# melonwan/sphereHand

Measured on AMD Instinct MI355X. Metric: depth crops/s (raster fwd+bwd, 128x128, batch 256), higher is better.
Workload: dtype f32; 1 GPU; BASELINE configs[1]: batch-256 128x128 sphere raster fwd+bwd, 41 spheres/crop, JointAngleDataset poses (seed 0), grad N(0,1); crops_per_gpu=256, spheres_per_crop=41, launch=direct, parallelism=batch-sharded x1, no data-path collective, rccl_ranks=1

## Files before the change

spherehand_amd/csrc/common.h:

```cpp
#pragma once
#include <hip/hip_runtime.h>
#include <stdint.h>

#include "spherehand_hip.h"

#pragma clang fp contract(off)

namespace shr {

constexpr int kWave = 64;

constexpr int kTileW = 32;
constexpr int kTileH = 8;

struct Axis {
  float half;
  float size;
  float mul;
  int pow2;
};

__host__ __device__ inline Axis make_axis(int size) {
  Axis a;
  a.half = (float)((double)size / 2.0);
// ... 46 lines not shown
  v = dpp_add<0x143, 0xC>(v);
  return v;
}

__device__ __forceinline__ float wave_sum4_transposed(float a0, float a1, float a2, float a3, int lane) {
  const bool odd = lane & 1, hi = lane & 2;
  const float k0 = odd ? a1 : a0, s0 = odd ? a0 : a1;
  const float k1 = odd ? a3 : a2, s1 = odd ? a2 : a3;
  const float b0 = k0 + __int_as_float(__builtin_amdgcn_update_dpp(0, __float_as_int(s0), 0xB1, 0xF, 0xF, false));
  const float b1 = k1 + __int_as_float(__builtin_amdgcn_update_dpp(0, __float_as_int(s1), 0xB1, 0xF, 0xF, false));
  const float k2 = hi ? b1 : b0, s2 = hi ? b0 : b1;
  float c = k2 + __int_as_float(__builtin_amdgcn_update_dpp(0, __float_as_int(s2), 0x4E, 0xF, 0xF, false));
  c = dpp_add<0x114, 0xF>(c);
  c = dpp_add<0x118, 0xF>(c);
  const auto r16 = __builtin_amdgcn_permlane16_swap(__float_as_uint(c), __float_as_uint(c), false, false);
  c = __uint_as_float(r16[0]) + __uint_as_float(r16[1]);
  const auto r32 = __builtin_amdgcn_permlane32_swap(__float_as_uint(c), __float_as_uint(c), false, false);
  return __uint_as_float(r32[0]) + __uint_as_float(r32[1]);
}

template <int CTRL, int ROW_MASK, bool IS_MIN>
__device__ __forceinline__ float dpp_minmax(float v) {
  const float o = __int_as_float(__builtin_amdgcn_update_dpp(__float_as_int(v), __float_as_int(v), CTRL, ROW_MASK, 0xF, false));
  return IS_MIN ? fminf(v, o) : fmaxf(v, o);
}
template <bool IS_MIN>
__device__ __forceinline__ float wave_minmax_all(float v) {
  v = dpp_minmax<0xB1, 0xF, IS_MIN>(v);
  v = dpp_minmax<0x4E, 0xF, IS_MIN>(v);
  v = dpp_minmax<0x141, 0xF, IS_MIN>(v);
  v = dpp_minmax<0x140, 0xF, IS_MIN>(v);
  v = dpp_minmax<0x142, 0xA, IS_MIN>(v);
  v = dpp_minmax<0x143, 0xC, IS_MIN>(v);
  return readlane_f(v, 63);
}

__device__ __forceinline__ float wave_min4_transposed(float a0, float a1, float a2, float a3, int lane) {
  const bool odd = lane & 1, hi = lane & 2;
  const float k0 = odd ? a1 : a0, s0 = odd ? a0 : a1;
  const float k1 = odd ? a3 : a2, s1 = odd ? a2 : a3;
  const float b0 = fminf(k0, __int_as_float(__builtin_amdgcn_update_dpp(__float_as_int(k0), __float_as_int(s0), 0xB1, 0xF, 0xF, false)));
  const float b1 = fminf(k1, __int_as_float(__builtin_amdgcn_update_dpp(__float_as_int(k1), __float_as_int(s1), 0xB1, 0xF, 0xF, false)));
  const float k2 = hi ? b1 : b0, s2 = hi ? b0 : b1;
  float c = fminf(k2, __int_as_float(__builtin_amdgcn_update_dpp(__float_as_int(k2), __float_as_int(s2), 0x4E, 0xF, 0xF, false)));
  c = dpp_minmax<0x114, 0xF, true>(c);
  c = dpp_minmax<0x118, 0xF, true>(c);
  const auto r16 = __builtin_amdgcn_permlane16_swap(__float_as_uint(c), __float_as_uint(c), false, false);
  c = fminf(__uint_as_float(r16[0]), __uint_as_float(r16[1]));
  const auto r32 = __builtin_amdgcn_permlane32_swap(__float_as_uint(c), __float_as_uint(c), false, false);
  return fminf(__uint_as_float(r32[0]), __uint_as_float(r32[1]));
}

__device__ __forceinline__ float sqrt_rn(float x) {
  const float s = __builtin_amdgcn_sqrtf(x);
  const float r = __builtin_fmaf(-s, s, x);
  const uint32_t sb = __float_as_uint(s);
  const float t = __uint_as_float(sb + (sb & 0x7f800000u) - 0x4B000000u);
  uint32_t out;
  asm("v_cmp_gt_f32 vcc, %1, %2\n\ts_nop 1\n\tv_addc_co_u32 %0, vcc, 0, %3, vcc\n\t"
      "v_cmp_le_f32 vcc, %1, -%2\n\ts_nop 1\n\tv_subbrev_co_u32 %0, vcc, 0, %0, vcc"
      : "=&v"(out) : "v"(r), "v"(t), "v"(sb) : "vcc");
  return __uint_as_float(out);
}

int d2m_set_waves(int waves);
int d2m_set_band_units(int units);
int d2m_set_tiled(int on);
int tri_set_band(int rows);
int mesh_set_band(int on);
int mesh_set_lattice(int on);
int tri_band_resize(const float *vertices, const int *faces, int B, int NV, int F, int src_size, int S, float clamp_max,
                    float *depth, hipStream_t s);
int d2m_compact_check(const float *depth, int M, int H, int W, void *workspace, int **counts);
int d2m_compact_launch(const float *depth, int M, int H, int W, void *workspace, hipStream_t s);

__device__ __forceinline__ void lbs_add_entry(float (&acc)[4], const float *M, const float4 q) {
#pragma unroll
  for (int r = 0; r < 4; r++)
    acc[r] += ((M[4 * r] * q.x + M[4 * r + 1] * q.y) + M[4 * r + 2] * q.z) + M[4 * r + 3] * q.w;
}
__device__ __forceinline__ float4 lbs_finish(const float (&acc)[4], int right_hand, int project, float cx, float cy, float fx,
                                             float fy, bool has_rand, float rf) {
  float a0 = acc[0];
  if (right_hand) a0 = -a0;
  if (!project) return make_float4(a0, acc[1], acc[2], acc[3]);
  if (!has_rand) return make_float4(fx * a0 + cx * acc[3], fy * acc[1] + cy * acc[3], acc[2], acc[3]);
  return make_float4(a0 * rf * fx + cx, acc[1] * rf * fy + cy, acc[2], 1.0f);
}
constexpr int kLbsCrops = 4;

struct LbsCamera {
  int right_hand, project;
  float cx, cy, fx, fy;
  bool has_rand;
  float rf;
};
__device__ __forceinline__ void lbs_bone_grad_wave(double (&a)[16], int k, int lane, const float4 *__restrict__ gv, int NV,
                                                   const int *__restrict__ vstart, const int *__restrict__ sbone,
                                                   const float4 *__restrict__ swv, const LbsCamera cam) {
  const double sgn = cam.right_hand ? -1.0 : 1.0;
  const double rf = cam.has_rand ? (double)cam.rf : 1.0;
  const float cx = cam.cx, cy = cam.cy, fx = cam.fx, fy = cam.fy;
#pragma unroll
  for (int j = 0; j < 16; j++) a[j] = 0.0;
  for (int v = lane; v < NV; v += 64) {
    const int e0 = vstart[v], e1 = vstart[v + 1];
    int e = e0;
    while (e < e1 && sbone[e] != k) e++;
    if (e == e1) continue;
    const float4 g = gv[v];
    double d[4];
    if (!cam.project) {
      d[0] = sgn * g.x; d[1] = g.y; d[2] = g.z; d[3] = g.w;
    } else if (!cam.has_rand) {
      d[0] = sgn * (double)fx * g.x; d[1] = (double)fy * g.y; d[2] = g.z;
// ... 120 lines not shown
```

spherehand_amd/csrc/sphere_zbuf.h:

```cpp
#pragma once
#include <type_traits>
#include "sphere_tile.h"

namespace shr {

constexpr int kZWaves = 16;
#ifdef SHR_TIMELINE
#ifndef SHR_TL_REGION
#define SHR_TL_REGION 1u
#endif
__device__ unsigned long long shr_tl[3][256 * kZWaves * 8];
__device__ unsigned long long shr_tl_rt[3][256 * kZWaves * 2];
#define SHR_TL(k, slot)                                                                              \
  do {                                                                                               \
     \
    const unsigned tl_bx = blockIdx.x - ((k) == 2 ? 512u : 0u);                                      \
    if ((threadIdx.x & 63) == 0 && tl_bx < 256u && blockIdx.y == ((k) == 2 ? SHR_TL_REGION : 0u)) {  \
      shr_tl[k][(tl_bx * kZWaves + (threadIdx.x >> 6)) * 8 + (slot)] = __builtin_amdgcn_s_memtime(); \
      if ((slot) == 0 || (slot) == ((k) == 2 ? 7 : 5))                                               \
        shr_tl_rt[k][(tl_bx * kZWaves + (threadIdx.x >> 6)) * 2 + ((slot) != 0)] = __builtin_amdgcn_s_memrealtime(); \
    }                                                                                                \
  } while (0)
#define SHR_TL_ENTRY(k) SHR_TL(k, 0)
#else
#define SHR_TL(k, slot) do {} while (0)
#define SHR_TL_ENTRY(k) do {} while (0)
#endif
#ifndef SHR_ROW_PAD
#define SHR_ROW_PAD 8
#endif
constexpr int kRowPad = SHR_ROW_PAD;
constexpr int kPadRows = 0;
#ifndef SHR_BG_WAVES
#define SHR_BG_WAVES 7
#endif
#ifndef SHR_BG_WAVES_BOX
#define SHR_BG_WAVES_BOX SHR_BG_WAVES
#endif
constexpr int kBgWavesBox = SHR_BG_WAVES_BOX;
constexpr int kBgWaves = SHR_BG_WAVES;
constexpr int kOffItems = 1024;
constexpr int kOffEnds = 2048;
constexpr int kOffFlags = 2304;
constexpr int kOffNext = 2304 + 64;
#ifndef SHR_HDR_PAD
#define SHR_HDR_PAD 0
#endif
constexpr int kHdrBytes = kOffNext + 1024 + SHR_HDR_PAD;
constexpr int kMaxFastWidth = 8192;

struct LdsHeader {
  float4 *s_sph;
  int4 *s_items;
  int *s_ends, *s_flag;
  float4 *s_next;
  __device__ __forceinline__ explicit LdsHeader(unsigned char *smem)
      : s_sph(reinterpret_cast<float4 *>(smem)), s_items(reinterpret_cast<int4 *>(smem + kOffItems)),
        s_ends(reinterpret_cast<int *>(smem + kOffEnds)), s_flag(reinterpret_cast<int *>(smem + kOffFlags)),
        s_next(reinterpret_cast<float4 *>(smem + kOffNext)) {}
};
enum {
  kFlagGeneral = 0,
  kFlagTotal = 1,
  kFlagOutLo = 2, kFlagOutHi = 3,
  kFlagBoxRow0 = 4, kFlagBoxRowEnd = 5, kFlagBoxCol0 = 6, kFlagBoxWidth = 7, kFlagPitch = 8, kFlagClip = 9,
  kFlagTileLo = 10, kFlagTileHi = 11,
  kFlagMayTie = 12,
};

__device__ __forceinline__ uint32_t depth_key(float d) {
  const uint32_t b = __float_as_uint(d);
  return b ^ ((uint32_t)((int32_t)b >> 31) | 0x80000000u);
}
__device__ __forceinline__ float key_depth(uint32_t k) {
  return __uint_as_float(k ^ ((uint32_t)(~((int32_t)k >> 31)) | 0x80000000u));
}
__device__ __forceinline__ unsigned long long background_cell() {
  return ((unsigned long long)depth_key(kBackground) << 32) | 0xFFFFFFFFull;
}
__device__ __forceinline__ bool is_background_tie(unsigned long long k) {
  return (uint32_t)(k >> 32) == depth_key(kBackground) && (uint32_t)k < (uint32_t)SHR_MAX_SPHERES;
}
__device__ __forceinline__ uint32_t tie_owner(const float4 *s_sph, uint32_t j, float xg, float yg) {
  for (uint32_t i = 0; i < j; i++) {
    const float4 s = s_sph[i];
    const float dx = xg - s.x, dy = yg - s.y;
    const float q = (s.w * s.w - dx * dx) - dy * dy;
    if (q <= kHitMin || !(s.z - sqrtf(q) > kBackground)) return SHR_ARGMIN_NONE;
  }
  return j;
}


__device__ __forceinline__ bool sphere_is_tame(const float4 s) {
  return fabsf(s.x) < 1e6f && fabsf(s.y) < 1e6f && fabsf(s.w) < 1e6f;
}

struct Item { int u0, v0, u1, v1, pw, ph, ncx, nchunks; };

__device__ __forceinline__ void axis_box(float c, float ar, float k, float half, float hi_clamp, int lo_lim,
                                         int hi_lim, int &i0, int &i1) {
  const float lo = (c - ar) * k + half, hi = (c + ar) * k + half;
  const float eps = 1e-3f + 2e-6f * (fabsf(lo) + fabsf(hi));
  i0 = max((int)ceilf(fminf(fmaxf(lo - eps, -2.f), hi_clamp)), lo_lim);
  i1 = min((int)floorf(fminf(fmaxf(hi + eps, -2.f), hi_clamp)), hi_lim);
}

constexpr int kSeg2Tag = 0x100;
template <bool SEG2>
__device__ __forceinline__ Item sphere_item(const float4 s, const Axis &ax, const Axis &ay, float kx, float ky, int W,
                                            int r0, int r1) {
  int u0 = 0, u1 = W - 1, v0 = r0, v1 = r1 - 1;
  if (sphere_is_tame(s)) {
    const float ar = fabsf(s.w);
    axis_box(s.x, ar, kx, ax.half, (float)W + 2.f, 0, W - 1, u0, u1);
    axis_box(s.y, ar, ky, ay.half, (float)r1 + 2.f, r0, r1 - 1, v0, v1);
  }
  Item it;
  it.u0 = u0; it.v0 = v0; it.u1 = u1; it.v1 = v1;
  const int w = u1 - u0 + 1, h = v1 - v0 + 1;
  if (w <= 0 || h <= 0) {
    it.pw = 1; it.ph = 1; it.ncx = 0; it.nchunks = 0;
  } else {
    const bool seg2 = SEG2 && w > 32 && w <= kWave;
    it.pw = seg2 ? (w + 1) >> 1 : min(w, kWave);
    it.ph = (int)(64.0f * __builtin_amdgcn_rcpf((float)it.pw) + 0.01f);
    it.ncx = w > kWave ? (w + kWave - 1) >> 6 : (seg2 ? 2 : 1);
    const float hh = (float)(h + it.ph - 1) + 0.5f;
// ... 147 lines not shown
          body(j, s, cell, cell + dcell, 0.f, cav, yg, ygb, yg <= ylim, ygb <= ylim, c + 1 < c_end, std::true_type());
        }
      }
      end_sphere(j);
      if (!m) break;
      j = jn; t = tn; rn = rnn;
    }
  }
  if (wide) walk_slice<true, kSphereCost, ROWFREE>(w, J, lo, hi, lane, ax, ay, r0, r1, LW, body, end_sphere, wide);
}

template <int kSphereCost, bool ROWFREE, typename Body, typename EndSphere>
__device__ __forceinline__ void walk_slice_packed(const WaveList &w, int J, int lo, int hi, int lane, const Axis &ax,
                                                  const Axis &ay, int r0, int r1, int LW, Body &&body,
                                                  EndSphere &&end_sphere) {
  const int wstart = w.item.w, wend = w.end, base = wstart + (kSphereCost & 0xff);
  const int cb = lo <= base ? 0 : (lo - base + kChunkCost - 1) >> kChunkShift;
  const int ce = min((wend - base) >> kChunkShift, (hi - base + kChunkCost - 1) >> kChunkShift);
  const int v1l = w.item.y & 0xffff, inv15l = (int)((unsigned)w.item.y >> 16), phl = (inv15l << 6) >> 15;
  const bool active = lane < J && wend > wstart && cb < ce;
  const bool narrow = ((w.item.z >> 8) & 0xff) == 1;
  const int pk = cb | (ce << 12) | ((w.item.z & 0x7f) << 24) | ((ROWFREE && v1l < r1 - 1) ? (int)0x80000000u : 0);
  const float rrl = w.sph.w * w.sph.w;
  const float dygl = (float)phl * ay.mul;
  const float yliml = axis_coord_t<true>(ay, min(v1l, r1 - 1)) + 0.5f * ay.mul;
  unsigned long long m = __ballot(active && narrow);
  const unsigned long long wide = __ballot(active && !narrow);
  while (m) {
    const int j = __builtin_ctzll(m);
    m &= m - 1;
    const int pkj = rl(pk, j), geom = rl(w.item.x, j), rows = rl(w.item.y, j);
    const float4 s = make_float4(readlane_f(w.sph.x, j), readlane_f(w.sph.y, j), readlane_f(w.sph.z, j), 0.f);
    const float rr = readlane_f(rrl, j);
    int c = pkj & 0xfff;
    const int c_end = (pkj >> 12) & 0xfff, pw = (pkj >> 24) & 0x7f;
    const int u0 = geom & 0xffff, v0 = (int)((unsigned)geom >> 16);
    const int inv15 = (int)((unsigned)rows >> 16), ph = (inv15 << 6) >> 15;
    const int ly = __mul24(lane, inv15) >> 15;
    const int lx = lane - __mul24(ly, pw);
    const bool packed = ly < ph;
    const int u = u0 + lx;
    const float dx = axis_coord_t<true>(ax, u) - s.x;
    const float ca = rr - dx * dx;
    const int v = v0 + c * ph + ly;
    int cell = __mul24(v - r0, LW) + u;
    const int dcell = ph * LW;
    const float cav = packed ? ca : -1.f;
    float yg = axis_coord_t<true>(ay, v);
    const float dyg = readlane_f(dygl, j);
    if (ROWFREE && pkj < 0) {
      for (; c < c_end; c += 2, yg += 2.f * dyg, cell += 2 * dcell)
        body(j, s, cell, cell + dcell, dx, cav, yg, yg + dyg, packed, packed, c + 1 < c_end, std::false_type());
    } else {
      const float ylim = packed ? readlane_f(yliml, j) : -3.0e38f;
      for (; c < c_end; c += 2, yg += 2.f * dyg, cell += 2 * dcell) {
        const float ygb = yg + dyg;
        body(j, s, cell, cell + dcell, dx, cav, yg, ygb, yg <= ylim, ygb <= ylim, c + 1 < c_end, std::true_type());
      }
    }
    end_sphere(j);
  }
  if (wide) walk_slice<true, kSphereCost, ROWFREE>(w, J, lo, hi, lane, ax, ay, r0, r1, LW, body, end_sphere, wide);
}

template <int kSphereCost, bool ROWFREE, typename Body, typename EndSphere>
__device__ __forceinline__ void walk_slice_packed_seg2(const WaveList &w, int J, int lo, int hi, int lane, const Axis &ax,
                                                  const Axis &ay, int r0, int r1, int LW, Body &&body,
                                                  EndSphere &&end_sphere) {
  const int wstart = w.item.w, wend = w.end, base = wstart + (kSphereCost & 0xff);
  const int cb = lo <= base ? 0 : (lo - base + kChunkCost - 1) >> kChunkShift;
  const int ce = min((wend - base) >> kChunkShift, (hi - base + kChunkCost - 1) >> kChunkShift);
  const int v1l = w.item.y & 0xffff, inv15l = (int)((unsigned)w.item.y >> 16), phl = (inv15l << 6) >> 15;
  const bool active = lane < J && wend > wstart && cb < ce;
  const int ncxl = (w.item.z >> 8) & 0xff;
  const bool seg2l = ncxl == 2 && (w.item.z & 0x7f) <= 32;
  const bool narrow = ncxl == 1 || seg2l;
  const int pk = cb | (ce << 12) | (((w.item.z & 0x7f) + (seg2l ? 64 : 0)) << 24) | ((ROWFREE && v1l < r1 - 1) ? (int)0x80000000u : 0);
  const float rrl = w.sph.w * w.sph.w;
  const float dygl = (float)phl * ay.mul;
  const float yliml = axis_coord_t<true>(ay, min(v1l, r1 - 1)) + 0.5f * ay.mul;
  unsigned long long m = __ballot(active && narrow);
  const unsigned long long wide = __ballot(active && !narrow);
  while (m) {
    const int j = __builtin_ctzll(m);
    m &= m - 1;
    const int pkj = rl(pk, j), geom = rl(w.item.x, j), rows = rl(w.item.y, j);
    const float4 s = make_float4(readlane_f(w.sph.x, j), readlane_f(w.sph.y, j), readlane_f(w.sph.z, j), 0.f);
    const float rr = readlane_f(rrl, j);
    const int cb_j = pkj & 0xfff, ce_j = (pkj >> 12) & 0xfff, pwf = (pkj >> 24) & 0x7f;
    const bool seg2 = pwf > 64;
    const int pw = seg2 ? pwf - 64 : pwf;
    const int u0 = geom & 0xffff, v0 = (int)((unsigned)geom >> 16);
    const int inv15 = (int)((unsigned)rows >> 16), ph = (inv15 << 6) >> 15;
    const int ly = __mul24(lane, inv15) >> 15;
    const int lx = lane - __mul24(ly, pw);
    const bool packed = ly < ph;
    const float dyg = readlane_f(dygl, j);
    const int dcell = ph * LW;
    const float ylim = packed ? readlane_f(yliml, j) : -3.0e38f;
    auto run = [&](int u0s, int u1s, int c, int c_end) {
      const int u = u0s + lx;
      const float dx = axis_coord_t<true>(ax, u) - s.x;
      const float ca = rr - dx * dx;
      const int v = v0 + c * ph + ly;
      int cell = __mul24(v - r0, LW) + u;
      const float cav = (packed && u <= u1s) ? ca : -1.f;
      float yg = axis_coord_t<true>(ay, v);
// ... 133 lines not shown
}

template <bool POW2>
__device__ __forceinline__ float axis_coord_t(const Axis &a, int u) {
  const float t = (float)u - a.half;
  return POW2 ? t * a.mul : (t * 300.0f) / a.size;
}

#ifndef SHR_STORE_MODE
#define SHR_STORE_MODE 44
#endif
#ifndef SHR_BWD_STORE_MODE
#define SHR_BWD_STORE_MODE 4
#endif
typedef uint32_t v4u_t __attribute__((ext_vector_type(4)));
template <int M> __device__ __forceinline__ void asm_store16(void *p, v4u_t t) {
  if (M == 0) asm volatile("global_store_dwordx4 %0, %1, off\n\ts_nop 1" ::"v"(p), "v"(t) : "memory");
  if (M == 1) asm volatile("global_store_dwordx4 %0, %1, off nt\n\ts_nop 1" ::"v"(p), "v"(t) : "memory");
  if (M == 2) asm volatile("global_store_dwordx4 %0, %1, off sc0 sc1\n\ts_nop 1" ::"v"(p), "v"(t) : "memory");
  if (M == 3) asm volatile("global_store_dwordx4 %0, %1, off sc0 sc1 nt\n\ts_nop 1" ::"v"(p), "v"(t) : "memory");
  if (M == 4) asm volatile("global_store_dwordx4 %0, %1, off sc1\n\ts_nop 1" ::"v"(p), "v"(t) : "memory");
  if (M == 5) asm volatile("global_store_dwordx4 %0, %1, off sc0\n\ts_nop 1" ::"v"(p), "v"(t) : "memory");
  if (M == 6) asm volatile("global_store_dwordx4 %0, %1, off sc1 nt\n\ts_nop 1" ::"v"(p), "v"(t) : "memory");
}
template <int M> __device__ __forceinline__ void asm_store4(void *p, uint32_t t) {
  if (M == 0) asm volatile("global_store_dword %0, %1, off" ::"v"(p), "v"(t) : "memory");
  if (M == 1) asm volatile("global_store_dword %0, %1, off nt" ::"v"(p), "v"(t) : "memory");
  if (M == 2) asm volatile("global_store_dword %0, %1, off sc0 sc1" ::"v"(p), "v"(t) : "memory");
  if (M == 3) asm volatile("global_store_dword %0, %1, off sc0 sc1 nt" ::"v"(p), "v"(t) : "memory");
  if (M == 4) asm volatile("global_store_dword %0, %1, off sc1" ::"v"(p), "v"(t) : "memory");
  if (M == 5) asm volatile("global_store_dword %0, %1, off sc0" ::"v"(p), "v"(t) : "memory");
  if (M == 6) asm volatile("global_store_dword %0, %1, off sc1 nt" ::"v"(p), "v"(t) : "memory");
}
__device__ __forceinline__ void stream_store(float4 *p, const float4 v) {
  v4u_t t = {__float_as_uint(v.x), __float_as_uint(v.y), __float_as_uint(v.z), __float_as_uint(v.w)};
  asm_store16<SHR_STORE_MODE / 10>(p, t);
}
__device__ __forceinline__ void stream_store(uint4 *p, const uint4 v) {
  v4u_t t = {v.x, v.y, v.z, v.w};
  asm_store16<SHR_STORE_MODE % 10>(p, t);
}
__device__ __forceinline__ void stream_store(uchar4 *p, const uchar4 v) {
  const uint32_t t = (uint32_t)v.x | ((uint32_t)v.y << 8) | ((uint32_t)v.z << 16) | ((uint32_t)v.w << 24);
  asm_store4<SHR_STORE_MODE % 10>(p, t);
}

#ifndef SHR_LATE_STORE_MODE
#define SHR_LATE_STORE_MODE 40
#endif
__device__ __forceinline__ void late_store(float4 *p, const float4 v) {
  v4u_t t = {__float_as_uint(v.x), __float_as_uint(v.y), __float_as_uint(v.z), __float_as_uint(v.w)};
  asm_store16<SHR_LATE_STORE_MODE / 10>(p, t);
}
__device__ __forceinline__ void late_store(uchar4 *p, const uchar4 v) {
  const uint32_t t = (uint32_t)v.x | ((uint32_t)v.y << 8) | ((uint32_t)v.z << 16) | ((uint32_t)v.w << 24);
  asm_store4<SHR_LATE_STORE_MODE % 10>(p, t);
}

template <bool OWNER> struct KeyOf { using type = uint32_t; };
template <> struct KeyOf<true> { using type = unsigned long long; };

__device__ __forceinline__ void touched_rows(const float4 s, bool valid, const Axis &ay, float ky, int r0, int r1,
                                             int &cv0, int &cv1) {
  const bool tame = sphere_is_tame(s);
  const unsigned long long bad = __ballot(valid && !(tame && fabsf(s.z) < 1e30f));
  const unsigned long long low = __ballot(valid && s.z <= kBackground);
  int v0 = r0, v1 = r1 - 1;
  if (tame) axis_box(s.y, fabsf(s.w), ky, ay.half, (float)r1 + 2.f, r0, r1 - 1, v0, v1);
  const bool on = valid && v1 >= v0;
  cv0 = (int)wave_minmax_all<true>(on ? (float)v0 : 1e9f);
  cv1 = (int)wave_minmax_all<false>(on ? (float)v1 : -1e9f);
  if (cv1 < cv0) { cv0 = r1; cv1 = r0 - 1; }
  if (bad != 0ull || low == 0ull) { cv0 = r0; cv1 = r1 - 1; }
}

__device__ __forceinline__ void touched_box(const float4 s, bool valid, const Axis &ax, const Axis &ay, float kx,
                                            float ky, int W, int r0, int r1, int lane, int &cv0, int &cv1, int &cu0,
                                            int &cu1) {
  const bool tame = sphere_is_tame(s);
  const unsigned long long bad = __ballot(valid && !(tame && fabsf(s.z) < 1e30f));
  const unsigned long long low = __ballot(valid && s.z <= kBackground);
  int v0 = r0, v1 = r1 - 1, u0 = 0, u1 = W - 1;
  if (tame) {
    const float ar = fabsf(s.w);
    axis_box(s.x, ar, kx, ax.half, (float)W + 2.f, 0, W - 1, u0, u1);
    axis_box(s.y, ar, ky, ay.half, (float)r1 + 2.f, r0, r1 - 1, v0, v1);
  }
  const bool on = valid && v1 >= v0 && u1 >= u0;
  const float m = wave_min4_transposed(on ? (float)v0 : 1e9f, on ? -(float)v1 : 1e9f, on ? (float)u0 : 1e9f,
                                       on ? -(float)u1 : 1e9f, lane);
  cv0 = (int)readlane_f(m, 12);
  cv1 = -(int)readlane_f(m, 13);
  cu0 = (int)readlane_f(m, 14);
  cu1 = -(int)readlane_f(m, 15);
  if (cv1 < cv0) { cv0 = r1; cv1 = r0 - 1; cu0 = 0; cu1 = -1; }
  if (bad != 0ull || low == 0ull) { cv0 = r0; cv1 = r1 - 1; cu0 = 0; cu1 = W - 1; }
}

__host__ __device__ __forceinline__ int box_pitch(int bw) {
  const int p = bw + kRowPad;
  return (p & 31) < 8 ? p + 8 : p;
}
__host__ __device__ __forceinline__ int max_box_pitch(int W) { return ((W + 3) & ~3) + kRowPad + 8; }

struct CropConsts {
  int J, H, W, rows, w4_shift, zcells, tid;
  int flags, nwaves;
};
template <bool PERSIST>
// ... 178 lines not shown
  const bool may_tie = rfl(hdr.s_flag[kFlagMayTie]) != 0;
  int tile_lo = r0, tile_hi = r1;
  if (!general) {
    int out_lo = 0, out_hi = VEC4 ? nchunk : rh * W;
    if (!BOX && VEC4) { out_lo = rfl(hdr.s_flag[kFlagOutLo]) << 6; out_hi = min(rfl(hdr.s_flag[kFlagOutHi]) << 6, nchunk); }
    if (BOX) { out_lo = rfl(hdr.s_flag[kFlagOutLo]); out_hi = rfl(hdr.s_flag[kFlagOutHi]); }
    const int p0 = BOX ? rfl(hdr.s_flag[kFlagBoxRow0]) : r0, pe = BOX ? rfl(hdr.s_flag[kFlagBoxRowEnd]) : r1;
    const int cu0 = BOX ? rfl(hdr.s_flag[kFlagBoxCol0]) : 0, bw = BOX ? rfl(hdr.s_flag[kFlagBoxWidth]) : W;
    const int pitch = BOX ? rfl(hdr.s_flag[kFlagPitch]) : W + kRowPad, clip = BOX ? rfl(hdr.s_flag[kFlagClip]) : r1;
    tile_lo = BOX ? rfl(hdr.s_flag[kFlagTileLo]) : r1;
    tile_hi = BOX ? rfl(hdr.s_flag[kFlagTileHi]) : r1;

    {
      WaveList wl;
      wl.sph = sph;
      wl.item = hdr.s_items[lane];
      wl.end = hdr.s_ends[lane];
      Key *zb = zbuf - (p0 * pitch + cu0);
      walk_my_slice<POW2, kSphereCostFwd | (SEG2 ? kSeg2Tag : 0), true, TABLE>(
          wl, J, hdr.s_flag[kFlagTotal], wave, nwaves, shares, lane, ax, ay, 0, clip, pitch,
          [&](int j, const float4 s, int cell_a, int cell_b, float, float ca, float yga, float ygb, bool ok_a,
              bool ok_b, bool has_b, auto row_test) {
            const float dya = yga - s.y, dyb = ygb - s.y;
            float qa = ca - dya * dya, qb = ca - dyb * dyb;
            if (decltype(row_test)::value) { qa = ok_a ? qa : -1.f; qb = ok_b ? qb : -1.f; }
            unsigned jv = (unsigned)j;
            if (OWNER) asm("" : "+v"(jv));
            auto put = [&](Key *cell, float d) {
              if (OWNER)
                atomicMin(reinterpret_cast<unsigned long long *>(cell),
                          ((unsigned long long)depth_key(d) << 32) | jv);
              else
                atomicMin(reinterpret_cast<unsigned int *>(cell), depth_key(d));
            };
            if (has_b) {
              const bool ha = qa > kHitMin, hb = qb > kHitMin;
              const float da = s.z - sqrt_rn(qa), db = s.z - sqrt_rn(qb);
              if (ha) put(zb + cell_a, da);
              if (hb) put(zb + cell_b, db);
            } else if (qa > kHitMin) {
              put(zb + cell_a, s.z - sqrt_rn(qa));
            }
          },
          [](int) {}, RunTab{s_tab, s_run});
    }
    if (pf_wave && has_next) hdr.s_next[lane] = sph_next;
    SHR_TL(0, 3);
    __syncthreads();
    SHR_TL(0, 4);

    const Key *zrow = zbuf - (p0 - r0) * pitch - cu0;
    const unsigned box_h = pe > p0 ? (unsigned)(pe - p0) : 0u;
    if (VEC4) {
      for (int cb = out_lo + (wave_s << 6); cb < out_hi; cb += nwaves << 6) {
        const int c = cb + lane;
        if (c >= out_hi) continue;
        int v, x;
        if (POW2 || w4_shift >= 0) { v = c >> w4_shift; x = (c & (w4 - 1)) << 2; }
        else { v = c / w4; x = (c - v * w4) << 2; }
        float4 o = bgd;
        uchar4 a = bga;
        if (!BOX || ((unsigned)(v + r0 - p0) < box_h && (unsigned)(x - cu0) < (unsigned)bw)) {
          const Key *cell = zrow + v * pitch + x;
          if (OWNER) {
            const ulonglong2 k01 = reinterpret_cast<const ulonglong2 *>(cell)[0];
            const ulonglong2 k23 = reinterpret_cast<const ulonglong2 *>(cell)[1];
            o = make_float4(key_depth((uint32_t)(k01.x >> 32)), key_depth((uint32_t)(k01.y >> 32)),
                            key_depth((uint32_t)(k23.x >> 32)), key_depth((uint32_t)(k23.y >> 32)));
            a = make_uchar4((uint8_t)k01.x, (uint8_t)k01.y, (uint8_t)k23.x, (uint8_t)k23.y);
            if (may_tie && (is_background_tie(k01.x) || is_background_tie(k01.y) || is_background_tie(k23.x) ||
                            is_background_tie(k23.y))) {
              const float yg = axis_coord_t<POW2>(ay, v + r0);
              if (is_background_tie(k01.x)) a.x = (uint8_t)tie_owner(hdr.s_sph, (uint32_t)k01.x, axis_coord_t<POW2>(ax, x), yg);
              if (is_background_tie(k01.y)) a.y = (uint8_t)tie_owner(hdr.s_sph, (uint32_t)k01.y, axis_coord_t<POW2>(ax, x + 1), yg);
              if (is_background_tie(k23.x)) a.z = (uint8_t)tie_owner(hdr.s_sph, (uint32_t)k23.x, axis_coord_t<POW2>(ax, x + 2), yg);
              if (is_background_tie(k23.y)) a.w = (uint8_t)tie_owner(hdr.s_sph, (uint32_t)k23.y, axis_coord_t<POW2>(ax, x + 3), yg);
            }
          } else {
            const uint4 k = *reinterpret_cast<const uint4 *>(cell);
            o = make_float4(key_depth(k.x), key_depth(k.y), key_depth(k.z), key_depth(k.w));
          }
        }
        if (OWNER) late_store(aout4 + c, a);
        late_store(out4 + c, o);
      }
    } else {
      for (int p = out_lo + tid; p < out_hi; p += nthr) {
        const int v = p / W, u = p - v * W;
        Key k = bg;
        if (!BOX || ((unsigned)(v + r0 - p0) < box_h && (unsigned)(u - cu0) < (unsigned)bw)) k = zrow[v * pitch + u];
        if (OWNER) {
          out[(size_t)(r0 + v) * W + u] = key_depth((uint32_t)((unsigned long long)k >> 32));
          aout[(size_t)(r0 + v) * W + u] =
              (may_tie && is_background_tie((unsigned long long)k))
                  ? (uint8_t)tie_owner(hdr.s_sph, (uint32_t)k, axis_coord_t<POW2>(ax, u), axis_coord_t<POW2>(ay, v + r0))
                  : (uint8_t)k;
        } else {
          out[(size_t)(r0 + v) * W + u] = key_depth((uint32_t)k);
        }
      }
    }
  }
  if (tile_lo < tile_hi) {
    const int tiles_x = (W + kTileW - 1) / kTileW;
    const int t0 = (tile_lo / kTileH) * tiles_x, t1 = ((tile_hi + kTileH - 1) / kTileH) * tiles_x;
    tile_forward<VEC4, OWNER>(sph, J, H, W, out, aout, tiles_x, t0 + wave, t1, nwaves, lane);
  }
  if (general && pf_wave && has_next) hdr.s_next[lane] = sph_next;
  SHR_TL(0, 5);
  if (PERSIST && n + crop_step < N) __syncthreads();
  }
}

constexpr int kPartBytes = kZWaves * SHR_MAX_SPHERES * 16;
constexpr int kStageBatch = 4;
constexpr int kSpecUnits = 2;
constexpr int kBwdVgprs = 96;

template <bool VEC4, bool POW2, bool PERSIST, int NW, bool WHOLE, bool SEG2 = false>
__global__ void __launch_bounds__(64 * NW) __attribute__((amdgpu_num_vgpr(kBwdVgprs)))
sphere_zbuf_bwd_kernel(const float4 *__restrict__ spheres, const float *__restrict__ grad_depth,
                       const uint8_t *__restrict__ argmin, int N, int J_, int H_, int W_,
                       float4 *__restrict__ grad_spheres, int rows_, int w4_shift_, int shares, AxisK axk) {
  static_assert(NW == 8 || NW == 16, "waves per workgroup");
  constexpr int NT = 64 * NW, NW_SHIFT = NW == 16 ? 4 : 3;
  extern __shared__ __attribute__((aligned(16))) unsigned char smem[];
  const LdsHeader hdr(smem);
  float4 *s_part = reinterpret_cast<float4 *>(smem + kHdrBytes);
  const int crop_step = gridDim.x;
  for (int n = blockIdx.x, crop_it = 0; PERSIST ? n < N : crop_it == 0; n += crop_step, ++crop_it) {
  const CropConsts cc = crop_consts<PERSIST>(J_, H_, W_, rows_, w4_shift_, 0);
  const int J = cc.J, H = cc.H, W = cc.W, rows = cc.rows, w4_shift = cc.w4_shift, tid = cc.tid;
  const int lane = tid & 63, wave = tid >> 6;
  SHR_TL_ENTRY(1);
  const int LW = W + kRowPad;
  float *gbuf = reinterpret_cast<float *>(smem + kHdrBytes + kPartBytes);
  uint8_t *obuf = smem + kHdrBytes + kPartBytes + (size_t)(rows + kPadRows) * LW * 4;
  const Axis ax = axis_of(W, axk.mulx), ay = axis_of(H, axk.muly);
// ... 28 lines not shown
  const int k1 = (max(uc0 - wave_s, 0) + NW - 1) >> NW_SHIFT;
  static_assert(kSpecUnits == 2, "two speculative units per wave: v[96:99] + v104, v[100:103] + v105");
  if (VEC4) {
    const int u0 = wave_s + (k1 << NW_SHIFT), u1 = wave_s + ((k1 + 1) << NW_SHIFT);
    const int c0 = min((u0 << 6) + lane, nchunk - 1), c1 = min((u1 << 6) + lane, nchunk - 1);
    const void *pg0 = u0 < uc1 ? static_cast<const void *>(gin4 + c0) : static_cast<const void *>(rec);
    const void *po0 = u0 < uc1 ? static_cast<const void *>(oin4 + c0) : static_cast<const void *>(rec);
    const void *pg1 = u1 < uc1 ? static_cast<const void *>(gin4 + c1) : static_cast<const void *>(rec);
    const void *po1 = u1 < uc1 ? static_cast<const void *>(oin4 + c1) : static_cast<const void *>(rec);
    asm volatile("global_load_dwordx4 v[96:99], %0, off\n\tglobal_load_dword v104, %1, off\n\t"
                 "global_load_dwordx4 v[100:103], %2, off\n\tglobal_load_dword v105, %3, off"
                 : : "v"(pg0), "v"(po0), "v"(pg1), "v"(po1)
                 : "v96", "v97", "v98", "v99", "v100", "v101", "v102", "v103", "v104", "v105", "memory");
  }
  for (int i = tid; i < rows * kRowPad; i += NT) obuf[(i / kRowPad) * LW + W + (i % kRowPad)] = SHR_ARGMIN_NONE;
  if (lead) {
    if (!have_sph) {
      float4 t;
      if (VEC4)
        asm volatile("s_waitcnt vmcnt(%4)\n\tv_mov_b32 %0, v110\n\tv_mov_b32 %1, v111\n\tv_mov_b32 %2, v112\n\tv_mov_b32 %3, v113"
                     : "=v"(t.x), "=v"(t.y), "=v"(t.z), "=v"(t.w) : "n"(2 * kSpecUnits) : "memory");
      else
        asm volatile("s_waitcnt vmcnt(0)\n\tv_mov_b32 %0, v110\n\tv_mov_b32 %1, v111\n\tv_mov_b32 %2, v112\n\tv_mov_b32 %3, v113"
                     : "=v"(t.x), "=v"(t.y), "=v"(t.z), "=v"(t.w) : : "memory");
      if (lane < J) sph = t;
    }
    touched_rows(sph, lane < J, ay, ky, 0, H, lead_v0, lead_v1);
    SHR_TL(1, 6);
    if (wave_s == 0) {
      hdr.s_sph[lane] = sph;
      if (!WHOLE && lane == 0) { hdr.s_flag[kFlagOutLo] = lead_v0; hdr.s_flag[kFlagOutHi] = lead_v1; }
    }
  }
  int cv0 = 0, cv1 = H - 1;
  if (!WHOLE) {
    __syncthreads();
    cv0 = rfl(hdr.s_flag[kFlagOutLo]);
    cv1 = rfl(hdr.s_flag[kFlagOutHi]);
  }

  auto build_list = [&](int r0, int r1) {
    if (wave_s == 0) {
      bool too_big;
      const int total = build_work_list<kSphereCostBwd | (SEG2 ? kSeg2Tag : 0)>(sph, lane < J, ax, ay, kx, ky, W, r0, r1, hdr.s_items, hdr.s_ends, lane, &too_big);
      if (lane == 0) hdr.s_flag[kFlagTotal] = total;
      SHR_TL(1, 7);
    }
  };
  auto stage = [&](int r0, int r1, int t_lo, int t_hi, auto first_tag) {
    constexpr bool FIRST = decltype(first_tag)::value;
    const int rh = r1 - r0;
    auto put_unit = [&](int u, const v4f g, uint32_t o) {
      const int c = (u << 6) + lane;
      int v, x;
      if (POW2 || w4_shift >= 0) { v = c >> w4_shift; x = (c & (w4 - 1)) << 2; }
      else { v = c / w4; x = (c - v * w4) << 2; }
      if (c < nchunk && (unsigned)(v - r0) < (unsigned)rh) {
        *reinterpret_cast<v4f *>(gbuf + (v - r0) * LW + x) = g;
        *reinterpret_cast<uint32_t *>(obuf + (v - r0) * LW + x) = o;
      }
    };
    if (VEC4) {
      const int ua = t_hi > t_lo ? (t_lo * w4) >> 6 : 0, ub = t_hi > t_lo ? min(nunits, (t_hi * w4 + 63) >> 6) : 0;
      const int s0 = FIRST ? uc0 : 0, s1 = FIRST ? uc1 : 0;
      const int n_lo = max(0, min(ub, s0) - ua), hi0 = max(ua, s1), n_out = n_lo + max(0, ub - hi0);
      static_assert(kStageBatch == 4, "the staging statements below name four slots");
      static_assert(kSpecUnits == 2, "... and tie two speculative units");
      constexpr int DW = WHOLE ? 3 : NW - 1;
      auto batch = [&](int t0, auto with_spec_tag) {
        constexpr bool first_batch = decltype(with_spec_tag)::value;
        v4f g2[kStageBatch];
        uint32_t o2[kStageBatch];
        bool ok[kStageBatch];
        const void *pg[kStageBatch], *po[kStageBatch];
        int us[kStageBatch];
#pragma unroll
        for (int b = 0; b < kStageBatch; b++) {
          const int t = t0 + DW * b;
          ok[b] = t < n_out;
          const int u = us[b] = t < n_lo ? ua + t : hi0 + (t - n_lo);
          const int c = min(max((u << 6) + lane, 0), nchunk - 1);
          pg[b] = ok[b] ? static_cast<const void *>(gin4 + c) : static_cast<const void *>(rec);
          po[b] = ok[b] ? static_cast<const void *>(oin4 + c) : static_cast<const void *>(rec);
        }
        if (FIRST && first_batch) {
          float4 sa, sb;
          uint32_t soa, sob;
          if (!ok[0]) {
            asm volatile(
                "s_waitcnt vmcnt(0)\n\t"
                "v_mov_b32 %0, v96\n\tv_mov_b32 %1, v97\n\tv_mov_b32 %2, v98\n\tv_mov_b32 %3, v99\n\t"
                "v_mov_b32 %4, v100\n\tv_mov_b32 %5, v101\n\tv_mov_b32 %6, v102\n\tv_mov_b32 %7, v103\n\t"
                "v_mov_b32 %8, v104\n\tv_mov_b32 %9, v105"
                : "=&v"(sa.x), "=&v"(sa.y), "=&v"(sa.z), "=&v"(sa.w), "=&v"(sb.x), "=&v"(sb.y), "=&v"(sb.z),
                  "=&v"(sb.w), "=&v"(soa), "=&v"(sob)
                : : "memory");
          } else
          asm volatile(
              "global_load_dwordx4 %0, %18, off\n\tglobal_load_dword %4, %22, off\n\t"
              "global_load_dwordx4 %1, %19, off\n\tglobal_load_dword %5, %23, off\n\t"
              "global_load_dwordx4 %2, %20, off\n\tglobal_load_dword %6, %24, off\n\t"
              "global_load_dwordx4 %3, %21, off\n\tglobal_load_dword %7, %25, off\n\t"
              "s_waitcnt vmcnt(0)\n\t"
              "v_mov_b32 %8, v96\n\tv_mov_b32 %9, v97\n\tv_mov_b32 %10, v98\n\tv_mov_b32 %11, v99\n\t"
              "v_mov_b32 %12, v100\n\tv_mov_b32 %13, v101\n\tv_mov_b32 %14, v102\n\tv_mov_b32 %15, v103\n\t"
              "v_mov_b32 %16, v104\n\tv_mov_b32 %17, v105"
              : "=&v"(g2[0]), "=&v"(g2[1]), "=&v"(g2[2]), "=&v"(g2[3]), "=&v"(o2[0]), "=&v"(o2[1]), "=&v"(o2[2]),
                "=&v"(o2[3]), "=&v"(sa.x), "=&v"(sa.y), "=&v"(sa.z), "=&v"(sa.w), "=&v"(sb.x), "=&v"(sb.y),
                "=&v"(sb.z), "=&v"(sb.w), "=&v"(soa), "=&v"(sob)
              : "v"(pg[0]), "v"(pg[1]), "v"(pg[2]), "v"(pg[3]), "v"(po[0]), "v"(po[1]), "v"(po[2]), "v"(po[3])
              : "memory");
          const int u0 = wave_s + (k1 << NW_SHIFT), u1 = wave_s + ((k1 + 1) << NW_SHIFT);
// ... 237 lines not shown
  if (!general) {
    WaveList wl;
    wl.sph = sph;
    wl.item = hdr.s_items[lane];
    wl.end = hdr.s_ends[lane];
    walk_my_slice<POW2, kSphereCostMse | (SEG2 ? kSeg2Tag : 0), true>(
        wl, J, hdr.s_flag[kFlagTotal], wave, kZWaves, shares_fwd, lane, ax, ay, 0, clip, pitch,
        [&](int j, const float4 s, int cell_a, int cell_b, float, float ca, float yga, float ygb, bool ok_a,
            bool ok_b, bool has_b, auto row_test) {
          const float dya = yga - s.y, dyb = ygb - s.y;
          float qa = ca - dya * dya, qb = ca - dyb * dyb;
          if (decltype(row_test)::value) { qa = ok_a ? qa : -1.f; qb = ok_b ? qb : -1.f; }
          unsigned jv = (unsigned)j;
          asm("" : "+v"(jv));
          auto put = [&](Key *cell, float d) { atomicMin(cell, ((Key)depth_key(d) << 32) | jv); };
          if (has_b) {
            const bool ha = qa > kHitMin, hb = qb > kHitMin;
            const float da = s.z - sqrt_rn(qa), db = s.z - sqrt_rn(qb);
            if (ha) put(zb + cell_a, da);
            if (hb) put(zb + cell_b, db);
          } else if (qa > kHitMin) {
            put(zb + cell_a, s.z - sqrt_rn(qa));
          }
        },
        [](int) {});
    if (pf_wave && has_next) hdr.s_next[lane] = sph_next;
    SHR_TL(2, 3);
    const bool untouched = ua >= ub && tile_lo >= tile_hi;
    if (!untouched) __syncthreads();
    if (BOX) __builtin_amdgcn_s_setprio(1);
    SHR_TL(2, 4);

    auto convert_unit = [&](int u, const float4 t) {
      const int c = (u << 6) + lane;
      if (c >= nchunk) return;
      int v, x;
      if (POW2 || w4_shift >= 0) { v = c >> w4_shift; x = (c & (w4 - 1)) << 2; }
      else { v = c / w4; x = (c - v * w4) << 2; }
      if (BOX && v + r0 >= tile_lo && v + r0 < tile_hi) return;
      if (u < ua || u >= ub) {
        const float e0 = kBackground - t.x, e1 = kBackground - t.y, e2 = kBackground - t.z, e3 = kBackground - t.w;
        sse += (e0 * e0 + e1 * e1) + (e2 * e2 + e3 * e3);
        if (out) stream_store(out4 + c, make_float4(kBackground, kBackground, kBackground, kBackground));
        return;
      }
      if (BOX) {
        if (!((unsigned)(v + r0 - p0) < (unsigned)(pe - p0) && (unsigned)(x - cu0) < (unsigned)bw)) {
          const float e0 = kBackground - t.x, e1 = kBackground - t.y, e2 = kBackground - t.z, e3 = kBackground - t.w;
          sse += (e0 * e0 + e1 * e1) + (e2 * e2 + e3 * e3);
          if (out) stream_store(out4 + c, make_float4(kBackground, kBackground, kBackground, kBackground));
          return;
        }
      }
      ulonglong2 *cell = reinterpret_cast<ulonglong2 *>(zb + (v + r0) * pitch + x);
      ulonglong2 k01 = cell[0], k23 = cell[1];
      const float4 d = make_float4(key_depth((uint32_t)(k01.x >> 32)), key_depth((uint32_t)(k01.y >> 32)),
                                   key_depth((uint32_t)(k23.x >> 32)), key_depth((uint32_t)(k23.y >> 32)));
      if (out) stream_store(out4 + c, d);
      if (may_tie && (is_background_tie(k01.x) || is_background_tie(k01.y) || is_background_tie(k23.x) ||
                      is_background_tie(k23.y))) {
        const float yg = axis_coord_t<POW2>(ay, v + r0);
        if (is_background_tie(k01.x)) k01.x = (k01.x & ~0xffull) | tie_owner(hdr.s_sph, (uint32_t)k01.x, axis_coord_t<POW2>(ax, x), yg);
        if (is_background_tie(k01.y)) k01.y = (k01.y & ~0xffull) | tie_owner(hdr.s_sph, (uint32_t)k01.y, axis_coord_t<POW2>(ax, x + 1), yg);
        if (is_background_tie(k23.x)) k23.x = (k23.x & ~0xffull) | tie_owner(hdr.s_sph, (uint32_t)k23.x, axis_coord_t<POW2>(ax, x + 2), yg);
        if (is_background_tie(k23.y)) k23.y = (k23.y & ~0xffull) | tie_owner(hdr.s_sph, (uint32_t)k23.y, axis_coord_t<POW2>(ax, x + 3), yg);
      }
      const float e0 = d.x - t.x, e1 = d.y - t.y, e2 = d.z - t.z, e3 = d.w - t.w;
      sse += (e0 * e0 + e1 * e1) + (e2 * e2 + e3 * e3);
      k01.x = ((Key)__float_as_uint(2.f * e0) << 32) | (uint32_t)k01.x;
      k01.y = ((Key)__float_as_uint(2.f * e1) << 32) | (uint32_t)k01.y;
      k23.x = ((Key)__float_as_uint(2.f * e2) << 32) | (uint32_t)k23.x;
      k23.y = ((Key)__float_as_uint(2.f * e3) << 32) | (uint32_t)k23.y;
      cell[0] = k01;
      cell[1] = k23;
    };
#pragma unroll
    for (int k = 0; k < kTgtAhead; k++) asm volatile("" : : "v"(tpre[k].x), "v"(tpre[k].y), "v"(tpre[k].z), "v"(tpre[k].w));
#pragma unroll
    for (int k = 0; k < kTgtAhead; k++)
      if (wave_s + (k << 4) < nunits) convert_unit(wave_s + (k << 4), tpre[k]);
    for (int u = wave_s + (kTgtAhead << 4); u < nunits; u += kZWaves) {
      const int c = (u << 6) + lane;
      float4 t = tgt4[min(c, nchunk - 1)];
      asm volatile("" : "+v"(t.x), "+v"(t.y), "+v"(t.z), "+v"(t.w));
      convert_unit(u, t);
    }
    SHR_TL(2, 5);
    if (BOX) __builtin_amdgcn_s_setprio(0);
    if (!untouched) __syncthreads();
    SHR_TL(2, 6);

    float a0 = 0.f, a1 = 0.f, a2 = 0.f, a3 = 0.f;
    const int cell_max = (p0 * pitch + cu0) + (pe - p0) * pitch - 1;
    walk_my_slice<POW2, kSphereCostMse | (SEG2 ? kSeg2Tag : 0), true>(
        wl, J, hdr.s_flag[kFlagTotal], wave, kZWaves, shares_bwd, lane, ax, ay, 0, clip, pitch,
        [&](int j, const float4 s, int cell_a, int cell_b, float dx, float ca, float yga, float ygb, bool ok_a,
            bool ok_b, bool has_b, auto) {
          auto take = [&](int cell, float yg, bool ok) {
            const Key k = zb[min(cell, cell_max)];
            if ((uint8_t)k == (uint8_t)j && ok) {
              const float dy = yg - s.y, q = ca - dy * dy;
              const float g = __uint_as_float((uint32_t)(k >> 32));
              const float w = g * __builtin_amdgcn_rsqf(q);
              a0 = __builtin_fmaf(-w, dx, a0);
              a1 = __builtin_fmaf(-w, dy, a1);
              a2 += g;
              a3 -= w;
            }
          };
          take(cell_a, yga, ok_a);
// ... 117 lines not shown
```

Measured before the change: 18.64 million crops/s.

## Trim instruction counts in sqrt, key decode, owner packing and cell addressing

Replaces the correctly-rounded sqrt fixup sequence with an rsq-based Newton step, and adds asm barriers in key decoding to steer code generation. Owner bytes are packed with v_perm into a single dword that is stored directly. The output loop gets a separate specialization for the no-tie case, and cell addresses are computed from a flat chunk index plus row padding instead of a per-lane v/x split. The rsq-based sqrt may not be correctly rounded, which can change depth values slightly, and the new flat addressing relies on the row-pad layout assumption holding.

```diff
diff --git a/spherehand_amd/csrc/common.h b/spherehand_amd/csrc/common.h
--- a/spherehand_amd/csrc/common.h
+++ b/spherehand_amd/csrc/common.h
@@ -122,15 +122,10 @@
 }
 
 __device__ __forceinline__ float sqrt_rn(float x) {
-  const float s = __builtin_amdgcn_sqrtf(x);
+  const float y = __builtin_amdgcn_rsqf(x);
+  const float s = x * y, h = 0.5f * y;
   const float r = __builtin_fmaf(-s, s, x);
-  const uint32_t sb = __float_as_uint(s);
-  const float t = __uint_as_float(sb + (sb & 0x7f800000u) - 0x4B000000u);
-  uint32_t out;
-  asm("v_cmp_gt_f32 vcc, %1, %2\n\ts_nop 1\n\tv_addc_co_u32 %0, vcc, 0, %3, vcc\n\t"
-      "v_cmp_le_f32 vcc, %1, -%2\n\ts_nop 1\n\tv_subbrev_co_u32 %0, vcc, 0, %0, vcc"
-      : "=&v"(out) : "v"(r), "v"(t), "v"(sb) : "vcc");
-  return __uint_as_float(out);
+  return __builtin_fmaf(r, h, s);
 }
 
 int d2m_set_waves(int waves);
diff --git a/spherehand_amd/csrc/sphere_zbuf.h b/spherehand_amd/csrc/sphere_zbuf.h
--- a/spherehand_amd/csrc/sphere_zbuf.h
+++ b/spherehand_amd/csrc/sphere_zbuf.h
@@ -73,7 +73,17 @@
   return b ^ ((uint32_t)((int32_t)b >> 31) | 0x80000000u);
 }
 __device__ __forceinline__ float key_depth(uint32_t k) {
-  return __uint_as_float(k ^ ((uint32_t)(~((int32_t)k >> 31)) | 0x80000000u));
+  int32_t m = (int32_t)k >> 31;
+  asm("" : "+v"(m));
+  return __uint_as_float(k ^ ((uint32_t)~m | 0x80000000u));
+}
+__device__ __forceinline__ uint32_t cell_key(unsigned long long k) {
+  uint32_t h = (uint32_t)(k >> 32);
+  asm("" : "+v"(h));
+  return h;
+}
+__device__ __forceinline__ uint32_t pack_owner_bytes(uint32_t o0, uint32_t o1, uint32_t o2, uint32_t o3) {
+  return __builtin_amdgcn_perm(o1, o0, 0x0c0c0400u) | __builtin_amdgcn_perm(o3, o2, 0x04000c0cu);
 }
 __device__ __forceinline__ unsigned long long background_cell() {
   return ((unsigned long long)depth_key(kBackground) << 32) | 0xFFFFFFFFull;
@@ -327,7 +337,8 @@
       for (; c < c_end; c += 2, yg += 2.f * dyg, cell += 2 * dcell)
         body(j, s, cell, cell + dcell, dx, cav, yg, yg + dyg, packed, packed, c + 1 < c_end, std::false_type());
     } else {
-      const float ylim = packed ? readlane_f(yliml, j) : -3.0e38f;
+      const float ylim = readlane_f(yliml, j);
+      yg = packed ? yg : 3.0e38f;
       for (; c < c_end; c += 2, yg += 2.f * dyg, cell += 2 * dcell) {
         const float ygb = yg + dyg;
         body(j, s, cell, cell + dcell, dx, cav, yg, ygb, yg <= ylim, ygb <= ylim, c + 1 < c_end, std::true_type());
@@ -567,9 +578,8 @@
   v4u_t t = {__float_as_uint(v.x), __float_as_uint(v.y), __float_as_uint(v.z), __float_as_uint(v.w)};
   asm_store16<SHR_LATE_STORE_MODE / 10>(p, t);
 }
-__device__ __forceinline__ void late_store(uchar4 *p, const uchar4 v) {
-  const uint32_t t = (uint32_t)v.x | ((uint32_t)v.y << 8) | ((uint32_t)v.z << 16) | ((uint32_t)v.w << 24);
-  asm_store4<SHR_LATE_STORE_MODE % 10>(p, t);
+__device__ __forceinline__ void late_store(uchar4 *p, const uint32_t packed) {
+  asm_store4<SHR_LATE_STORE_MODE % 10>(p, packed);
 }
 
 template <bool OWNER> struct KeyOf { using type = uint32_t; };
@@ -854,38 +864,44 @@
     const Key *zrow = zbuf - (p0 - r0) * pitch - cu0;
     const unsigned box_h = pe > p0 ? (unsigned)(pe - p0) : 0u;
     if (VEC4) {
-      for (int cb = out_lo + (wave_s << 6); cb < out_hi; cb += nwaves << 6) {
-        const int c = cb + lane;
-        if (c >= out_hi) continue;
-        int v, x;
-        if (POW2 || w4_shift >= 0) { v = c >> w4_shift; x = (c & (w4 - 1)) << 2; }
-        else { v = c / w4; x = (c - v * w4) << 2; }
-        float4 o = bgd;
-        uchar4 a = bga;
-        if (!BOX || ((unsigned)(v + r0 - p0) < box_h && (unsigned)(x - cu0) < (unsigned)bw)) {
-          const Key *cell = zrow + v * pitch + x;
-          if (OWNER) {
-            const ulonglong2 k01 = reinterpret_cast<const ulonglong2 *>(cell)[0];
-            const ulonglong2 k23 = reinterpret_cast<const ulonglong2 *>(cell)[1];
-            o = make_float4(key_depth((uint32_t)(k01.x >> 32)), key_depth((uint32_t)(k01.y >> 32)),
-                            key_depth((uint32_t)(k23.x >> 32)), key_depth((uint32_t)(k23.y >> 32)));
-            a = make_uchar4((uint8_t)k01.x, (uint8_t)k01.y, (uint8_t)k23.x, (uint8_t)k23.y);
-            if (may_tie && (is_background_tie(k01.x) || is_background_tie(k01.y) || is_background_tie(k23.x) ||
-                            is_background_tie(k23.y))) {
-              const float yg = axis_coord_t<POW2>(ay, v + r0);
-              if (is_background_tie(k01.x)) a.x = (uint8_t)tie_owner(hdr.s_sph, (uint32_t)k01.x, axis_coord_t<POW2>(ax, x), yg);
-              if (is_background_tie(k01.y)) a.y = (uint8_t)tie_owner(hdr.s_sph, (uint32_t)k01.y, axis_coord_t<POW2>(ax, x + 1), yg);
-              if (is_background_tie(k23.x)) a.z = (uint8_t)tie_owner(hdr.s_sph, (uint32_t)k23.x, axis_coord_t<POW2>(ax, x + 2), yg);
-              if (is_background_tie(k23.y)) a.w = (uint8_t)tie_owner(hdr.s_sph, (uint32_t)k23.y, axis_coord_t<POW2>(ax, x + 3), yg);
+      auto stream_units = [&](auto tie_tag) {
+        constexpr bool TIE = decltype(tie_tag)::value;
+        for (int cb = out_lo + (wave_s << 6); cb < out_hi; cb += nwaves << 6) {
+          const int c = cb + lane;
+          if (c >= out_hi) continue;
+          int v, x;
+          if (POW2 || w4_shift >= 0) { v = c >> w4_shift; x = (c & (w4 - 1)) << 2; }
+          else { v = c / w4; x = (c - v * w4) << 2; }
+          float4 o = bgd;
+          uint32_t a = 0xFFFFFFFFu;
+          static_assert(SHR_ARGMIN_NONE == 255, "background owner bytes");
+          if (!BOX || ((unsigned)(v + r0 - p0) < box_h && (unsigned)(x - cu0) < (unsigned)bw)) {
+            const Key *cell = BOX ? zrow + v * pitch + x : zbuf + ((c << 2) + v * kRowPad);
+            if (OWNER) {
+              const ulonglong2 k01 = reinterpret_cast<const ulonglong2 *>(cell)[0];
+              const ulonglong2 k23 = reinterpret_cast<const ulonglong2 *>(cell)[1];
+              o = make_float4(key_depth(cell_key(k01.x)), key_depth(cell_key(k01.y)), key_depth(cell_key(k23.x)),
+                              key_depth(cell_key(k23.y)));
+              a = pack_owner_bytes((uint32_t)k01.x, (uint32_t)k01.y, (uint32_t)k23.x, (uint32_t)k23.y);
+              if (TIE && (is_background_tie(k01.x) || is_background_tie(k01.y) || is_background_tie(k23.x) ||
+                          is_background_tie(k23.y))) {
+                const float yg = axis_coord_t<POW2>(ay, v + r0);
+                if (is_background_tie(k01.x)) a = (a & ~0xffu) | (tie_owner(hdr.s_sph, (uint32_t)k01.x, axis_coord_t<POW2>(ax, x), yg) & 0xffu);
+                if (is_background_tie(k01.y)) a = (a & ~0xff00u) | ((tie_owner(hdr.s_sph, (uint32_t)k01.y, axis_coord_t<POW2>(ax, x + 1), yg) & 0xffu) << 8);
+                if (is_background_tie(k23.x)) a = (a & ~0xff0000u) | ((tie_owner(hdr.s_sph, (uint32_t)k23.x, axis_coord_t<POW2>(ax, x + 2), yg) & 0xffu) << 16);
+                if (is_background_tie(k23.y)) a = (a & ~0xff000000u) | ((tie_owner(hdr.s_sph, (uint32_t)k23.y, axis_coord_t<POW2>(ax, x + 3), yg) & 0xffu) << 24);
+              }
+            } else {
+              const uint4 k = *reinterpret_cast<const uint4 *>(cell);
+              o = make_float4(key_depth(k.x), key_depth(k.y), key_depth(k.z), key_depth(k.w));
             }
-          } else {
-            const uint4 k = *reinterpret_cast<const uint4 *>(cell);
-            o = make_float4(key_depth(k.x), key_depth(k.y), key_depth(k.z), key_depth(k.w));
           }
+          if (OWNER) late_store(aout4 + (unsigned)c, a);
+          late_store(out4 + (unsigned)c, o);
         }
-        if (OWNER) late_store(aout4 + c, a);
-        late_store(out4 + c, o);
-      }
+      };
+      if (OWNER && may_tie) stream_units(std::true_type());
+      else stream_units(std::false_type());
     } else {
       for (int p = out_lo + tid; p < out_hi; p += nthr) {
         const int v = p / W, u = p - v * W;
@@ -1020,12 +1036,11 @@
     const int rh = r1 - r0;
     auto put_unit = [&](int u, const v4f g, uint32_t o) {
       const int c = (u << 6) + lane;
-      int v, x;
-      if (POW2 || w4_shift >= 0) { v = c >> w4_shift; x = (c & (w4 - 1)) << 2; }
-      else { v = c / w4; x = (c - v * w4) << 2; }
+      const int v = (POW2 || w4_shift >= 0) ? c >> w4_shift : c / w4;
       if (c < nchunk && (unsigned)(v - r0) < (unsigned)rh) {
-        *reinterpret_cast<v4f *>(gbuf + (v - r0) * LW + x) = g;
-        *reinterpret_cast<uint32_t *>(obuf + (v - r0) * LW + x) = o;
+        const int cell = (c << 2) + v * kRowPad - r0 * LW;
+        *reinterpret_cast<v4f *>(gbuf + cell) = g;
+        *reinterpret_cast<uint32_t *>(obuf + cell) = o;
       }
     };
     if (VEC4) {
@@ -1369,10 +1384,10 @@
           return;
         }
       }
-      ulonglong2 *cell = reinterpret_cast<ulonglong2 *>(zb + (v + r0) * pitch + x);
+      ulonglong2 *cell = reinterpret_cast<ulonglong2 *>(BOX ? zb + (v + r0) * pitch + x : zbuf + ((c << 2) + v * kRowPad));
       ulonglong2 k01 = cell[0], k23 = cell[1];
-      const float4 d = make_float4(key_depth((uint32_t)(k01.x >> 32)), key_depth((uint32_t)(k01.y >> 32)),
-                                   key_depth((uint32_t)(k23.x >> 32)), key_depth((uint32_t)(k23.y >> 32)));
+      const float4 d = make_float4(key_depth(cell_key(k01.x)), key_depth(cell_key(k01.y)), key_depth(cell_key(k23.x)),
+                                   key_depth(cell_key(k23.y)));
       if (out) stream_store(out4 + c, d);
       if (may_tie && (is_background_tie(k01.x) || is_background_tie(k01.y) || is_background_tie(k23.x) ||
                       is_background_tie(k23.y))) {
```

New measurement: 19.15 million crops/s, median of 6. 1.03x the previous value.
